# dusk-network/plonk

Hardware: NVIDIA H100
Metric: proofs/sec @ 2^16 gates (higher is better)
Workload: dtype u32 limbs (Fr 256-bit / Fp 384-bit Montgomery)

## Files before the change

plonk_b200/csrc/bigint.cuh:

```cuda
#pragma once
#include <stdint.h>

#if defined(__CUDACC__)
#define PB_HD __host__ __device__ __forceinline__
#define PB_D __device__ __forceinline__
#else
#define PB_HD inline
#define PB_D inline
#endif

#ifndef PB_SPLIT
#define PB_SPLIT 0
#endif

namespace pb {

#if defined(__CUDA_ARCH__)
#define PB_ASM2(name, ins)                                                         \
  PB_D uint32_t name(uint32_t a, uint32_t b) {                                     \
    uint32_t r;                                                                    \
    asm volatile(ins " %0, %1, %2;" : "=r"(r) : "r"(a), "r"(b));                   \
    return r;                                                                      \
  }
#define PB_ASM3(name, ins)                                                         \
// ... 81 lines not shown
#ifndef PB_FR_HYBRID
#define PB_FR_HYBRID 0
#endif
}
#if !defined(__CUDA_ARCH__)
#include <math.h>
#include <string.h>
#endif
namespace pb {
PB_HD double fma_rz(double a, double b, double c) {
#if defined(__CUDA_ARCH__)
  return __fma_rz(a, b, c);
#else
  return fma(a, b, c);
#endif
}
PB_HD uint64_t dbl_bits(double x) {
#if defined(__CUDA_ARCH__)
  return (uint64_t)__double_as_longlong(x);
#else
  uint64_t r;
  memcpy(&r, &x, 8);
  return r;
#endif
}
PB_HD double bits_dbl(uint32_t hi, uint32_t lo) {
#if defined(__CUDA_ARCH__)
  return __hiloint2double((int)hi, (int)lo);
#else
  const uint64_t r = ((uint64_t)hi << 32) | lo;
  double x;
  memcpy(&x, &r, 8);
  return x;
#endif
}

template <class P>
struct Field {
  static constexpr int N = P::N;
  uint32_t v[N];

  static PB_HD Field zero() {
    Field r;
#pragma unroll
    for (int i = 0; i < N; i++) r.v[i] = 0;
    return r;
  }
  static PB_HD Field one() {
    Field r;
#pragma unroll
    for (int i = 0; i < N; i++) r.v[i] = P::R1(i);
    return r;
  }
  static PB_HD Field r2() {
    Field r;
#pragma unroll
    for (int i = 0; i < N; i++) r.v[i] = P::R2(i);
    return r;
  }
  PB_HD bool is_zero() const {
    uint32_t x = 0;
#pragma unroll
    for (int i = 0; i < N; i++) x |= v[i];
    return x == 0;
  }
  PB_HD bool operator==(const Field& o) const {
    uint32_t x = 0;
#pragma unroll
    for (int i = 0; i < N; i++) x |= v[i] ^ o.v[i];
    return x == 0;
  }
  PB_HD bool operator!=(const Field& o) const { return !(*this == o); }

  static PB_HD void final_sub(uint32_t* r, const uint32_t* t, uint32_t hi) {
    uint32_t s[N];
    s[0] = sub_cc(t[0], P::MOD(0));
#pragma unroll
    for (int i = 1; i < N; i++) s[i] = subc_cc(t[i], P::MOD(i));
    uint32_t borrow = subc(hi, 0u);
    bool ge = (borrow == 0u);
#pragma unroll
    for (int i = 0; i < N; i++) r[i] = ge ? s[i] : t[i];
  }

  friend PB_HD Field operator+(const Field& a, const Field& b) {
    uint32_t t[N];
    t[0] = add_cc(a.v[0], b.v[0]);
#pragma unroll
    for (int i = 1; i < N; i++) t[i] = addc_cc(a.v[i], b.v[i]);
    uint32_t hi = addc(0u, 0u);
    Field r;
    final_sub(r.v, t, hi);
    return r;
  }
  friend PB_HD Field operator-(const Field& a, const Field& b) {
    uint32_t t[N];
    t[0] = sub_cc(a.v[0], b.v[0]);
#pragma unroll
    for (int i = 1; i < N; i++) t[i] = subc_cc(a.v[i], b.v[i]);
    uint32_t borrow = subc(0u, 0u);
    Field r;
    uint32_t m = borrow;
    r.v[0] = add_cc(t[0], P::MOD(0) & m);
#pragma unroll
    for (int i = 1; i < N - 1; i++) r.v[i] = addc_cc(t[i], P::MOD(i) & m);
    r.v[N - 1] = addc(t[N - 1], P::MOD(N - 1) & m);
    return r;
  }
  PB_HD Field neg() const { return zero() - *this; }
  PB_HD Field dbl() const { return *this + *this; }

  template <bool SPLIT, bool CIN, bool COUT>
  static PB_HD void link(uint32_t& lo, uint32_t& hi, uint32_t a, uint32_t b, uint32_t clo, uint32_t chi) {
    if (SPLIT)
      mad_pair_split<CIN, COUT>(lo, hi, a, b, clo, chi);
    else
      mad_pair<CIN, COUT>(lo, hi, a, b, clo, chi);
  }
  static PB_HD void mul_row(uint32_t* X, uint32_t* Y, const uint32_t* a, uint32_t bi) {
    constexpr bool S0 = (PB_SPLIT & 1) != 0, S1 = (PB_SPLIT & 2) != 0;
    Y[0] = add_cc(Y[0], X[1]);
#pragma unroll
    for (int k = 0; k < N - 2; k += 2) link<S0, true, true>(X[k], X[k + 1], a[k + 1], bi, X[k + 2], X[k + 3]);
    link<S0, true, false>(X[N - 2], X[N - 1], a[N - 1], bi, 0u, 0u);
    link<S1, false, true>(Y[0], Y[1], a[0], bi, Y[0], Y[1]);
#pragma unroll
    for (int j = 2; j < N; j += 2) link<S1, true, true>(Y[j], Y[j + 1], a[j], bi, Y[j], Y[j + 1]);
    X[N - 1] = addc(X[N - 1], 0u);
  }
  static PB_HD void acc_row(uint32_t* X, uint32_t* Y, const uint32_t* c, uint32_t di) {
    constexpr bool S0 = (PB_SPLIT & 1) != 0, S1 = (PB_SPLIT & 2) != 0;
    link<S0, false, true>(X[0], X[1], c[1], di, X[0], X[1]);
#pragma unroll
    for (int k = 2; k < N - 2; k += 2) link<S0, true, true>(X[k], X[k + 1], c[k + 1], di, X[k], X[k + 1]);
    link<S0, true, false>(X[N - 2], X[N - 1], c[N - 1], di, X[N - 2], X[N - 1]);
    link<S1, false, true>(Y[0], Y[1], c[0], di, Y[0], Y[1]);
#pragma unroll
    for (int j = 2; j < N; j += 2) link<S1, true, true>(Y[j], Y[j + 1], c[j], di, Y[j], Y[j + 1]);
    X[N - 1] = addc(X[N - 1], 0u);
  }
  static PB_HD void red_row(uint32_t* X , uint32_t* Y ) {
    constexpr bool S2 = (PB_SPLIT & 4) != 0, S3 = (PB_SPLIT & 8) != 0;
    const uint32_t m = mul_lo(Y[0], P::inv());
    link<S2, false, true>(X[0], X[1], P::MOD(1), m, X[0], X[1]);
#pragma unroll
    for (int k = 2; k < N - 2; k += 2) link<S2, true, true>(X[k], X[k + 1], P::MOD(k + 1), m, X[k], X[k + 1]);
    link<S2, true, false>(X[N - 2], X[N - 1], P::MOD(N - 1), m, X[N - 2], X[N - 1]);
    link<S3, false, true>(Y[0], Y[1], P::MOD(0), m, Y[0], Y[1]);
#pragma unroll
    for (int j = 2; j < N; j += 2) link<S3, true, true>(Y[j], Y[j + 1], P::MOD(j), m, Y[j], Y[j + 1]);
    X[N - 1] = addc(X[N - 1], 0u);
  }
  template <bool FIRST>
  static PB_HD void mont_row(uint32_t* X , uint32_t* Y ,
                             const uint32_t* a, uint32_t bi) {
    if (!FIRST) mul_row(X, Y, a, bi);
    red_row(X, Y);
  }

  friend PB_HD Field operator*(const Field& a, const Field& b) {
#if defined(__CUDA_ARCH__)
    if constexpr (P::HYBRID) return mul_hybrid(a, b);
#endif
    return mul_imad(a, b);
  }
  static PB_HD Field mul_imad(const Field& a, const Field& b) {
    uint32_t A[N], B[N];
    {
      const uint32_t bi = b.v[0];
#pragma unroll
      for (int j = 0; j < N; j += 2) {
        mul_pair(A[j], A[j + 1], a.v[j], bi);
        mul_pair(B[j], B[j + 1], a.v[j + 1], bi);
      }
      mont_row<true>(B, A, a.v, bi);
    }
#pragma unroll
    for (int i = 1; i < N - 1; i += 2) {
      mont_row<false>(A, B, a.v, b.v[i]);
      mont_row<false>(B, A, a.v, b.v[i + 1]);
    }
    mont_row<false>(A, B, a.v, b.v[N - 1]);
    uint32_t t[N];
    t[0] = add_cc(A[0], B[1]);
#pragma unroll
    for (int k = 1; k < N - 1; k++) t[k] = addc_cc(A[k], B[k + 1]);
    t[N - 1] = addc(A[N - 1], 0u);
    Field r;
    final_sub(r.v, t, 0u);
    return r;
  }
  template <int I>
  static PB_HD uint32_t sq_limb(const uint32_t* a, const uint32_t* a2, int k) {
    return k == I ? a[k] : (k == I + 1 ? (a[k] << 1) : a2[k]);
  }
  template <int I>
  static PB_HD void sqr_row(uint32_t* X, uint32_t* Y, const uint32_t* a, const uint32_t* a2) {
    constexpr bool S0 = (PB_SPLIT & 1) != 0, S1 = (PB_SPLIT & 2) != 0;
    const uint32_t bi = a[I];
    Y[0] = add_cc(Y[0], X[1]);
    constexpr int K0 = I & ~1;
#pragma unroll
    for (int k = 0; k < K0; k += 2) {
      X[k] = addc_cc(X[k + 2], 0u);
      X[k + 1] = addc_cc(X[k + 3], 0u);
    }
#pragma unroll
    for (int k = K0; k < N - 2; k += 2) link<S0, true, true>(X[k], X[k + 1], sq_limb<I>(a, a2, k + 1), bi, X[k + 2], X[k + 3]);
    link<S0, true, false>(X[N - 2], X[N - 1], sq_limb<I>(a, a2, N - 1), bi, 0u, 0u);
    constexpr int J0 = (I + 1) & ~1;
    if (J0 < N) {
      link<S1, false, true>(Y[J0], Y[J0 + 1], sq_limb<I>(a, a2, J0), bi, Y[J0], Y[J0 + 1]);
#pragma unroll
      for (int j = J0 + 2; j < N; j += 2) link<S1, true, true>(Y[j], Y[j + 1], sq_limb<I>(a, a2, j), bi, Y[j], Y[j + 1]);
      X[N - 1] = addc(X[N - 1], 0u);
    }
  }
  template <int I>
  static PB_HD void sqr_rows(uint32_t* A, uint32_t* B, const uint32_t* a, const uint32_t* a2) {
    if constexpr (I < N) {
      sqr_row<I>(A, B, a, a2);
      red_row(A, B);
      if constexpr (I + 1 < N) {
        sqr_row<I + 1>(B, A, a, a2);
        red_row(B, A);
      }
      sqr_rows<I + 2>(A, B, a, a2);
    }
  }
  PB_HD Field sqr() const {
#if defined(__CUDA_ARCH__)
    if constexpr (P::HYBRID && (P::MOD(N - 1) >> 30) == 0) return sqr_hybrid();
#endif
    if constexpr ((P::MOD(N - 1) >> 30) != 0) {
      return (*this) * (*this);
    } else {
      return sqr_half();
    }
  }
  PB_HD Field sqr_half() const {
    static_assert((P::MOD(N - 1) >> 30) == 0, "needs two spare bits in the top limb of the modulus");
    uint32_t a2[N];
    a2[0] = v[0] << 1;
#pragma unroll
    for (int k = 1; k < N; k++) a2[k] = (v[k] << 1) | (v[k - 1] >> 31);
    uint32_t A[N], B[N];
    {
      const uint32_t bi = v[0];
#pragma unroll
      for (int j = 0; j < N; j += 2) {
        mul_pair(A[j], A[j + 1], sq_limb<0>(v, a2, j), bi);
        mul_pair(B[j], B[j + 1], sq_limb<0>(v, a2, j + 1), bi);
      }
      red_row(B, A);
    }
    sqr_rows<1>(A, B, v, a2);
    uint32_t t[N];
    t[0] = add_cc(A[0], B[1]);
#pragma unroll
    for (int k = 1; k < N - 1; k++) t[k] = addc_cc(A[k], B[k + 1]);
    t[N - 1] = addc(A[N - 1], 0u);
    Field r;
    final_sub(r.v, t, 0u);
    return r;
  }

  static PB_HD Field mul2(const Field& a, const Field& b, const Field& c, const Field& d) {
#if defined(__CUDA_ARCH__)
    if constexpr (P::HYBRID) return mul2_hybrid(a, b, c, d);
#endif
    return mul2_imad(a, b, c, d);
  }
  static PB_HD Field mul2_imad(const Field& a, const Field& b, const Field& c, const Field& d) {
    static_assert((P::MOD(N - 1) >> 30) == 0, "mul2 needs two spare bits in the top limb of the modulus");
    uint32_t A[N], B[N];
    {
      const uint32_t bi = b.v[0];
#pragma unroll
      for (int j = 0; j < N; j += 2) {
        mul_pair(A[j], A[j + 1], a.v[j], bi);
        mul_pair(B[j], B[j + 1], a.v[j + 1], bi);
      }
      acc_row(B, A, c.v, d.v[0]);
      red_row(B, A);
    }
#pragma unroll
    for (int i = 1; i < N - 1; i += 2) {
      mul_row(A, B, a.v, b.v[i]);
      acc_row(A, B, c.v, d.v[i]);
      red_row(A, B);
      mul_row(B, A, a.v, b.v[i + 1]);
      acc_row(B, A, c.v, d.v[i + 1]);
      red_row(B, A);
    }
    mul_row(A, B, a.v, b.v[N - 1]);
    acc_row(A, B, c.v, d.v[N - 1]);
    red_row(A, B);
    uint32_t t[N];
    t[0] = add_cc(A[0], B[1]);
#pragma unroll
    for (int k = 1; k < N - 1; k++) t[k] = addc_cc(A[k], B[k + 1]);
    t[N - 1] = addc(A[N - 1], 0u);
    Field r;
    final_sub(r.v, t, 0u);
    return r;
  }
  static constexpr int L48 = (32 * N + 47) / 48;
  static constexpr int CUT_COL = (32 * N) / 48;
  static constexpr int CUT_SH = (32 * N) % 48;
  static constexpr int LAST_BITS = 32 * N - 48 * (L48 - 1);
  static PB_HD constexpr int npairs48(int k) { return k < 0 ? 0 : (k < L48 ? k + 1 : (k <= 2 * L48 - 2 ? 2 * L48 - 1 - k : 0)); }
  static PB_HD constexpr uint64_t col_off48(int k) {
    return (uint64_t)npairs48(k) * 0x4330000000000000ull + (uint64_t)npairs48(k - 1) * 0x4630000000000000ull;
  }
  static PB_HD uint32_t word_or_zero(const uint32_t* T, int k) { return k < 2 * N ? T[k] : 0u; }
  static PB_HD Field redc48(const uint32_t* T) {
    uint64_t c[2 * L48];
    const uint32_t gate = T[2 * N - 1] >> 30;
#pragma unroll
    for (int q = 0; q < L48; q++) {
      const uint32_t w0 = word_or_zero(T, 3 * q) | (q == 0 ? gate : 0u), w1 = word_or_zero(T, 3 * q + 1),
                     w2 = word_or_zero(T, 3 * q + 2);
      c[2 * q] = (uint64_t)w0 | ((uint64_t)(w1 & 0xffffu) << 32);
      c[2 * q + 1] = (uint64_t)((w1 >> 16) | (w2 << 16)) | ((uint64_t)(w2 >> 16) << 32);
    }
    const double C1 = 0x1p100, C2 = 0x1p100 + 0x1p52;
#pragma unroll
    for (int i = 0; i < L48; i++) {
      const uint32_t qlo = (uint32_t)c[i], qhi = (uint32_t)(c[i] >> 32);
      const uint64_t r = (uint64_t)qlo * P::inv48_lo();
      uint32_t rlo = (uint32_t)r, rhi = ((uint32_t)(r >> 32) + qlo * P::inv48_hi() + qhi * P::inv48_lo()) & 0xffffu;
      if (i == L48 - 1 && LAST_BITS < 48) {
        static_assert(LAST_BITS == 48 || LAST_BITS <= 32, "last step narrower than a word or a whole limb");
        rhi = 0;
        if (LAST_BITS < 32) rlo &= (1u << (LAST_BITS & 31)) - 1u;
      }
      const double m = bits_dbl(0x43300000u | rhi, rlo) - 0x1p52;
      double hi_prev = 0;
#pragma unroll
      for (int j = 0; j < L48; j++) {
        const double pj = (double)P::MOD48(j);
        const double hi = fma_rz(m, pj, C1);
        const double lo = fma_rz(m, pj, C2 - hi);
        if (j == 0)
          c[i] += dbl_bits(lo);
        else
          c[i + j] += dbl_bits(lo) + dbl_bits(hi_prev);
        hi_prev = hi;
      }
      c[i + L48] += dbl_bits(hi_prev);
      if (i < CUT_COL) c[i + 1] += (c[i] - col_off48(i)) >> 48;
    }
#pragma unroll
    for (int k = CUT_COL; k < 2 * L48; k++) c[k] -= col_off48(k);
#pragma unroll
    for (int k = CUT_COL; k < 2 * L48 - 1; k++) {
      c[k + 1] += c[k] >> 48;
      c[k] &= 0xffffffffffffull;
    }
    uint32_t t[N];
#pragma unroll
    for (int w = 0; w < N; w++) {
      const int s = CUT_SH + 32 * w, k = CUT_COL + s / 48, o = s % 48;
      if (o == 0)
        t[w] = (uint32_t)c[k];
      else if (o == 16)
        t[w] = (uint32_t)(c[k] >> 16);
      else
        t[w] = (uint32_t)(c[k] >> 32) | ((uint32_t)c[k + 1] << 16);
    }
    Field res;
    final_sub(res.v, t, 0u);
    return res;
  }
  static PB_HD void wide_top(uint32_t* T, const uint32_t* A, const uint32_t* B) {
    T[N] = add_cc(A[0], B[1]);
#pragma unroll
    for (int k = 1; k < N - 1; k++) T[N + k] = addc_cc(A[k], B[k + 1]);
    T[2 * N - 1] = addc(A[N - 1], 0u);
  }
  template <bool TWO>
  static PB_HD void wide_mul(uint32_t* T, const uint32_t* a, const uint32_t* b, const uint32_t* c, const uint32_t* d) {
    uint32_t A[N], B[N];
#pragma unroll
    for (int j = 0; j < N; j += 2) {
      mul_pair(A[j], A[j + 1], a[j], b[0]);
      mul_pair(B[j], B[j + 1], a[j + 1], b[0]);
    }
    if (TWO) acc_row(B, A, c, d[0]);
    T[0] = A[0];
#pragma unroll
    for (int i = 1; i < N; i += 2) {
      mul_row(A, B, a, b[i]);
      if (TWO) acc_row(A, B, c, d[i]);
      T[i] = B[0];
      if (i + 1 < N) {
        mul_row(B, A, a, b[i + 1]);
        if (TWO) acc_row(B, A, c, d[i + 1]);
        T[i + 1] = A[0];
      }
    }
    wide_top(T, A, B);
  }
  template <int I>
  static PB_HD void wide_sqr_rows(uint32_t* T, uint32_t* A, uint32_t* B, const uint32_t* a, const uint32_t* a2) {
    if constexpr (I < N) {
      sqr_row<I>(A, B, a, a2);
      T[I] = B[0];
      if constexpr (I + 1 < N) {
        sqr_row<I + 1>(B, A, a, a2);
        T[I + 1] = A[0];
      }
      wide_sqr_rows<I + 2>(T, A, B, a, a2);
    }
  }
  static PB_HD void wide_sqr(uint32_t* T, const uint32_t* v) {
    uint32_t a2[N];
    a2[0] = v[0] << 1;
#pragma unroll
    for (int k = 1; k < N; k++) a2[k] = (v[k] << 1) | (v[k - 1] >> 31);
    uint32_t A[N], B[N];
#pragma unroll
    for (int j = 0; j < N; j += 2) {
      mul_pair(A[j], A[j + 1], sq_limb<0>(v, a2, j), v[0]);
      mul_pair(B[j], B[j + 1], sq_limb<0>(v, a2, j + 1), v[0]);
    }
    T[0] = A[0];
    wide_sqr_rows<1>(T, A, B, v, a2);
    wide_top(T, A, B);
  }
  static PB_HD Field mul_hybrid(const Field& a, const Field& b) {
    uint32_t T[2 * N];
    wide_mul<false>(T, a.v, b.v, a.v, b.v);
    return redc48(T);
  }
  PB_HD Field sqr_hybrid() const {
    static_assert((P::MOD(N - 1) >> 30) == 0, "needs two spare bits in the top limb of the modulus");
    uint32_t T[2 * N];
    wide_sqr(T, v);
    return redc48(T);
  }
  static PB_HD Field mul2_hybrid(const Field& a, const Field& b, const Field& c, const Field& d) {
    static_assert((P::MOD(N - 1) >> 30) == 0, "needs two spare bits in the top limb of the modulus");
    uint32_t T[2 * N];
    wide_mul<true>(T, a.v, b.v, c.v, d.v);
    return redc48(T);
  }

  static PB_HD Field mul_sub(const Field& a, const Field& b, const Field& c, const Field& d) { return mul2(a, b, c.neg(), d); }


  PB_HD Field from_mont() const {
    Field o = zero();
    o.v[0] = 1;
    return (*this) * o;
  }
  PB_HD Field to_mont() const { return (*this) * r2(); }

  PB_HD Field pow(const uint32_t* e, int words) const {
    Field acc = one();
    bool started = false;
    for (int w = words - 1; w >= 0; w--) {
      for (int bit = 31; bit >= 0; bit--) {
        if (started) acc = acc.sqr();
        if ((e[w] >> bit) & 1u) {
          acc = started ? acc * (*this) : *this;
          started = true;
        }
      }
    }
    return acc;
  }
  PB_HD Field pow_u64(uint64_t e) const {
    uint32_t w[2] = {(uint32_t)e, (uint32_t)(e >> 32)};
    return pow(w, 2);
  }
  PB_HD Field inv() const {
    uint32_t e[N];
    e[0] = sub_cc(P::MOD(0), 2u);
#pragma unroll
    for (int i = 1; i < N; i++) e[i] = subc_cc(P::MOD(i), 0u);
    return pow(e, N);
  }
};

#define PB_LIMB_TABLE(name, n, ...)                     \
  static PB_HD constexpr uint32_t name(int i) {         \
    constexpr uint32_t T[n] = {__VA_ARGS__};            \
    return T[i];                                        \
  }

#if defined(__CUDACC__)
static __constant__ uint32_t c_fr_inv = 0xffffffffu;
#endif

struct FrParams {
  static constexpr int N = 8;
  static constexpr bool HYBRID = PB_FR_HYBRID != 0;
  static PB_HD constexpr uint64_t MOD48(int j) {
    constexpr uint64_t T[6] = {0xffff00000001ull, 0xfffe5bfeffffull, 0xd80553bda402ull, 0x3339d80809a1ull,
                               0xa753299d7d48ull, 0x73edull};
    return T[j];
  }
  static PB_HD constexpr uint32_t inv48_lo() { return 0xffffffffu; }
  static PB_HD constexpr uint32_t inv48_hi() { return 0xfffeu; }
  static PB_HD uint32_t inv() {
#if defined(__CUDA_ARCH__)
    return c_fr_inv;
#else
    return 0xffffffffu;
#endif
  }
  PB_LIMB_TABLE(MOD, 8, 0x00000001u, 0xffffffffu, 0xfffe5bfeu, 0x53bda402u, 0x09a1d805u, 0x3339d808u,
                0x299d7d48u, 0x73eda753u)
  PB_LIMB_TABLE(R1, 8, 0xfffffffeu, 0x00000001u, 0x00034802u, 0x5884b7fau, 0xecbc4ff5u, 0x998c4fefu,
                0xacc5056fu, 0x1824b159u)
  PB_LIMB_TABLE(R2, 8, 0xf3f29c6du, 0xc999e990u, 0x87925c23u, 0x2b6cedcbu, 0x7254398fu, 0x05d31496u,
                0x9f59ff11u, 0x0748d9d9u)
};

struct FpParams {
  static constexpr int N = 12;
  static constexpr bool HYBRID = PB_FP_HYBRID != 0;
  static PB_HD constexpr uint64_t MOD48(int j) {
    constexpr uint64_t T[8] = {0xffffffffaaabull, 0xb153ffffb9feull, 0xf6241eabfffeull, 0x6730d2a0f6b0ull,
                               0x4b84f38512bfull, 0x434bacd76477ull, 0xe69a4b1ba7b6ull, 0x1a0111ea397full};
    return T[j];
  }
  static PB_HD constexpr uint32_t inv48_lo() { return 0xfffcfffdu; }
  static PB_HD constexpr uint32_t inv48_hi() { return 0xfffcu; }
  static PB_HD uint32_t inv() { return 0xfffcfffdu; }
  PB_LIMB_TABLE(MOD, 12, 0xffffaaabu, 0xb9feffffu, 0xb153ffffu, 0x1eabfffeu, 0xf6b0f624u, 0x6730d2a0u,
                0xf38512bfu, 0x64774b84u, 0x434bacd7u, 0x4b1ba7b6u, 0x397fe69au, 0x1a0111eau)
  PB_LIMB_TABLE(R1, 12, 0x0002fffdu, 0x76090000u, 0xc40c0002u, 0xebf4000bu, 0x53c758bau, 0x5f489857u,
                0x70525745u, 0x77ce5853u, 0xa256ec6du, 0x5c071a97u, 0xfa80e493u, 0x15f65ec3u)
  PB_LIMB_TABLE(R2, 12, 0x1c341746u, 0xf4df1f34u, 0x09d104f1u, 0x0a76e6a6u, 0x4c95b6d5u, 0x8de5476cu,
                0x939d83c0u, 0x67eb88a9u, 0xb519952du, 0x9a793e85u, 0x92cae3aau, 0x11988fe5u)
};

typedef Field<FrParams> Fr;
typedef Field<FpParams> Fp;

}
```

plonk_b200/csrc/ecntt.cu:

```cuda
#include "common.cuh"
#include "ecntt.cuh"

namespace pb {

int get_twiddles(int logm, bool inverse, cudaStream_t st, const uint4** out);
Fr ntt_size_inv(int log_n);

namespace {

PB_D Fp ec_ld_fp(const uint4* q) {
  const uint4 a = q[0], b = q[1], c = q[2];
  Fp f;
  f.v[0] = a.x; f.v[1] = a.y; f.v[2] = a.z; f.v[3] = a.w;
  f.v[4] = b.x; f.v[5] = b.y; f.v[6] = b.z; f.v[7] = b.w;
  f.v[8] = c.x; f.v[9] = c.y; f.v[10] = c.z; f.v[11] = c.w;
  return f;
}
PB_D void ec_st_fp(uint4* q, const Fp& f) {
  q[0] = make_uint4(f.v[0], f.v[1], f.v[2], f.v[3]);
  q[1] = make_uint4(f.v[4], f.v[5], f.v[6], f.v[7]);
  q[2] = make_uint4(f.v[8], f.v[9], f.v[10], f.v[11]);
}
PB_D G1Xyzz ec_ld_xyzz(const uint4* p, size_t i) {
  G1Xyzz a;
  a.x = ec_ld_fp(p + 12 * i);
  a.y = ec_ld_fp(p + 12 * i + 3);
  a.zz = ec_ld_fp(p + 12 * i + 6);
  a.zzz = ec_ld_fp(p + 12 * i + 9);
  return a;
}
PB_D void ec_st_xyzz(uint4* p, size_t i, const G1Xyzz& a) {
  ec_st_fp(p + 12 * i, a.x);
  ec_st_fp(p + 12 * i + 3, a.y);
  ec_st_fp(p + 12 * i + 6, a.zz);
  ec_st_fp(p + 12 * i + 9, a.zzz);
}
PB_D Fr ec_ld_fr(const uint4* p, size_t i) {
  const uint4 a = p[2 * i], b = p[2 * i + 1];
  Fr f;
  f.v[0] = a.x; f.v[1] = a.y; f.v[2] = a.z; f.v[3] = a.w;
  f.v[4] = b.x; f.v[5] = b.y; f.v[6] = b.z; f.v[7] = b.w;
  return f;
}

__global__ void k_ec_load(const uint4* aff, size_t n, uint4* A) {
  const size_t i = (size_t)blockIdx.x * blockDim.x + threadIdx.x;
  if (i >= n) return;
  G1Affine p;
  p.x = ec_ld_fp(aff + 6 * i);
  p.y = ec_ld_fp(aff + 6 * i + 3);
  ec_st_xyzz(A, i, G1Xyzz::from_affine(p));
}

__global__ void __launch_bounds__(128) k_ec_stage(uint4* A, size_t n, int s, const uint4* tw) {
  const size_t t = (size_t)blockIdx.x * blockDim.x + threadIdx.x;
  if (t >= n / 2) return;
  const size_t len = n >> s, half = len >> 1;
  const size_t blk = t / half, j = t % half, i0 = blk * len + j, ex = j << s;
  G1Xyzz a = ec_ld_xyzz(A, i0), b = ec_ld_xyzz(A, i0 + half);
  ec_butterfly(a, b, ec_ld_fr(tw, ex), ex == 0);
  ec_st_xyzz(A, i0, a);
  ec_st_xyzz(A, i0 + half, b);
}

struct EcScalar {
  uint32_t k[8];
};
__global__ void __launch_bounds__(128) k_ec_finish(const uint4* A, size_t n, int log_n, EcScalar n_inv, uint4* out) {
  const size_t i = (size_t)blockIdx.x * blockDim.x + threadIdx.x;
  if (i >= n) return;
  const G1Affine r = xyzz_to_affine(xyzz_mul(ec_ld_xyzz(A, i), n_inv.k, 8));
  const size_t o = ec_bitrev((unsigned)i, log_n);
  ec_st_fp(out + 6 * o, r.x);
  ec_st_fp(out + 6 * o + 3, r.y);
}

}

int lagrange_key_dev(const uint4* d_in, int log_n, uint4* d_out, cudaStream_t st) {
  if (log_n < 0 || log_n > 28) return fail(PB200_ERR_INVALID_DOMAIN, "group-element NTT size");
  const size_t n = (size_t)1 << log_n;
  uint4* A = nullptr;
  PB_CUDA(cudaMalloc((void**)&A, n * 192));
  struct Free {
    uint4* p;
    ~Free() { cudaFree(p); }
  } guard{A};
  PB_LAUNCH(k_ec_load, div_up(n, 128), 128, 0, st, d_in, n, A);
  if (log_n > 0) {
    const uint4* tw = nullptr;
    PB_TRY(get_twiddles(log_n, true, st, &tw));
    for (int s = 0; s < log_n; s++) PB_LAUNCH(k_ec_stage, div_up(n / 2, 128), 128, 0, st, A, n, s, tw);
  }
  EcScalar ninv;
  const Fr c = ntt_size_inv(log_n).from_mont();
  for (int i = 0; i < 8; i++) ninv.k[i] = c.v[i];
  PB_LAUNCH(k_ec_finish, div_up(n, 128), 128, 0, st, (const uint4*)A, n, log_n, ninv, d_out);
  PB_CUDA(cudaGetLastError());
  PB_CUDA(stream_wait(st));
  return 0;
}

}
```

plonk_b200/csrc/g1.cuh:

```cuda
#pragma once
#include "bigint.cuh"

namespace pb {

struct G1Affine {
  Fp x, y;
  PB_HD bool is_inf() const { return x.is_zero() && y.is_zero(); }
};

struct G1Xyzz {
  Fp x, y, zz, zzz;
  static PB_HD G1Xyzz identity() {
    G1Xyzz r;
    r.x = Fp::zero();
    r.y = Fp::zero();
    r.zz = Fp::zero();
    r.zzz = Fp::zero();
    return r;
  }
  PB_HD bool is_inf() const { return zz.is_zero(); }
  static PB_HD G1Xyzz from_affine(const G1Affine& p) {
    G1Xyzz r;
    if (p.is_inf()) return identity();
    r.x = p.x;
    r.y = p.y;
    r.zz = Fp::one();
    r.zzz = Fp::one();
    return r;
  }
  PB_HD G1Xyzz neg() const {
    G1Xyzz r = *this;
    r.y = y.neg();
    return r;
  }
};

PB_HD G1Xyzz xyzz_dbl_affine(const Fp& x1, const Fp& y1) {
  G1Xyzz r;
  if (y1.is_zero()) return G1Xyzz::identity();
  Fp u = y1.dbl();
  Fp v = u.sqr();
  Fp w = u * v;
  Fp s = x1 * v;
  Fp xx = x1.sqr();
  Fp m = xx.dbl() + xx;
  r.x = m.sqr() - s.dbl();
  r.y = Fp::mul_sub(m, s - r.x, w, y1);
  r.zz = v;
  r.zzz = w;
  return r;
}

PB_HD G1Xyzz xyzz_dbl(const G1Xyzz& p) {
  if (p.is_inf()) return p;
  if (p.y.is_zero()) return G1Xyzz::identity();
  G1Xyzz r;
  Fp u = p.y.dbl();
  Fp v = u.sqr();
  Fp w = u * v;
  Fp s = p.x * v;
  Fp xx = p.x.sqr();
  Fp m = xx.dbl() + xx;
  r.x = m.sqr() - s.dbl();
  r.y = Fp::mul_sub(m, s - r.x, w, p.y);
  r.zz = v * p.zz;
  r.zzz = w * p.zzz;
  return r;
}

PB_HD void xyzz_madd(G1Xyzz& acc, const Fp& x2, const Fp& y2) {
  if (acc.is_inf()) {
    acc.x = x2;
    acc.y = y2;
    acc.zz = Fp::one();
    acc.zzz = Fp::one();
    return;
  }
  Fp u2 = x2 * acc.zz;
  Fp s2 = y2 * acc.zzz;
  Fp p = u2 - acc.x;
  Fp r = s2 - acc.y;
  if (p.is_zero()) {
    if (r.is_zero())
      acc = xyzz_dbl_affine(x2, y2);
    else
      acc = G1Xyzz::identity();
    return;
  }
  Fp pp = p.sqr();
  Fp ppp = p * pp;
  Fp q = acc.x * pp;
  Fp x3 = r.sqr() - ppp - q.dbl();
  Fp y3 = Fp::mul_sub(r, q - x3, acc.y, ppp);
  acc.x = x3;
  acc.y = y3;
  acc.zz = acc.zz * pp;
  acc.zzz = acc.zzz * ppp;
}

PB_HD void xyzz_add(G1Xyzz& acc, const G1Xyzz& o) {
  if (o.is_inf()) return;
  if (acc.is_inf()) {
    acc = o;
    return;
  }
  Fp u1 = acc.x * o.zz;
  Fp u2 = o.x * acc.zz;
  Fp s1 = acc.y * o.zzz;
  Fp s2 = o.y * acc.zzz;
  Fp p = u2 - u1;
  Fp r = s2 - s1;
  if (p.is_zero()) {
    if (r.is_zero())
      acc = xyzz_dbl(acc);
    else
      acc = G1Xyzz::identity();
    return;
  }
  Fp pp = p.sqr();
  Fp ppp = p * pp;
  Fp q = u1 * pp;
  Fp x3 = r.sqr() - ppp - q.dbl();
  Fp y3 = Fp::mul_sub(r, q - x3, s1, ppp);
  acc.x = x3;
  acc.y = y3;
  acc.zz = acc.zz * o.zz * pp;
  acc.zzz = acc.zzz * o.zzz * ppp;
}

PB_HD G1Xyzz xyzz_mul(const G1Xyzz& p, const uint32_t* k, int words) {
  G1Xyzz acc = G1Xyzz::identity();
  bool started = false;
  for (int w = words - 1; w >= 0; w--) {
    for (int bit = 31; bit >= 0; bit--) {
      if (started) acc = xyzz_dbl(acc);
      if ((k[w] >> bit) & 1u) {
        if (started) {
          xyzz_add(acc, p);
        } else {
          acc = p;
          started = true;
        }
      }
    }
  }
  return acc;
}

PB_HD G1Affine xyzz_to_affine(const G1Xyzz& p) {
  G1Affine r;
  if (p.is_inf()) {
    r.x = Fp::zero();
    r.y = Fp::zero();
    return r;
  }
  Fp i = (p.zz * p.zzz).inv();
  Fp izz = i * p.zzz;
  Fp izzz = i * p.zz;
  r.x = p.x * izz;
  r.y = p.y * izzz;
  return r;
}

}
```

plonk_b200/csrc/msm.cu:

```cuda
#include <algorithm>
#include <atomic>
#include <vector>

#include "common.cuh"
#include "fp_inv.cuh"
#include "g1.cuh"
#include "host_field.h"

struct pb200_srs {
  size_t n_points;
  int c;
  int W;
  uint4* table;
};

namespace pb {

static constexpr int kGroup = 8;
static constexpr unsigned kHeavyMin = 32, kHeavyFactor = 4;
static constexpr unsigned kHeavyChunk = 256, kHeavyChunkWide = 1024;

PB_D G1Affine ld_affine(const uint4* p, size_t i) {
  const uint4* q = p + 6 * i;
  uint4 a0 = __ldg(q), a1 = __ldg(q + 1), a2 = __ldg(q + 2), b0 = __ldg(q + 3), b1 = __ldg(q + 4), b2 = __ldg(q + 5);
  G1Affine r;
  r.x.v[0] = a0.x; r.x.v[1] = a0.y; r.x.v[2] = a0.z; r.x.v[3] = a0.w;
  r.x.v[4] = a1.x; r.x.v[5] = a1.y; r.x.v[6] = a1.z; r.x.v[7] = a1.w;
  r.x.v[8] = a2.x; r.x.v[9] = a2.y; r.x.v[10] = a2.z; r.x.v[11] = a2.w;
  r.y.v[0] = b0.x; r.y.v[1] = b0.y; r.y.v[2] = b0.z; r.y.v[3] = b0.w;
  r.y.v[4] = b1.x; r.y.v[5] = b1.y; r.y.v[6] = b1.z; r.y.v[7] = b1.w;
  r.y.v[8] = b2.x; r.y.v[9] = b2.y; r.y.v[10] = b2.z; r.y.v[11] = b2.w;
  return r;
}
PB_D void st_fp(uint4* q, const Fp& f) {
  q[0] = make_uint4(f.v[0], f.v[1], f.v[2], f.v[3]);
  q[1] = make_uint4(f.v[4], f.v[5], f.v[6], f.v[7]);
  q[2] = make_uint4(f.v[8], f.v[9], f.v[10], f.v[11]);
}
PB_D Fp ld_fp(const uint4* q) {
  uint4 a = q[0], b = q[1], c = q[2];
  Fp f;
  f.v[0] = a.x; f.v[1] = a.y; f.v[2] = a.z; f.v[3] = a.w;
  f.v[4] = b.x; f.v[5] = b.y; f.v[6] = b.z; f.v[7] = b.w;
  f.v[8] = c.x; f.v[9] = c.y; f.v[10] = c.z; f.v[11] = c.w;
  return f;
}
PB_D void st_affine(uint4* p, size_t i, const G1Affine& a) {
  st_fp(p + 6 * i, a.x);
  st_fp(p + 6 * i + 3, a.y);
}
PB_D void st_xyzz(uint4* p, size_t i, const G1Xyzz& a) {
  st_fp(p + 12 * i, a.x);
  st_fp(p + 12 * i + 3, a.y);
  st_fp(p + 12 * i + 6, a.zz);
  st_fp(p + 12 * i + 9, a.zzz);
}
PB_D G1Xyzz ld_xyzz(const uint4* p, size_t i) {
  G1Xyzz a;
  a.x = ld_fp(p + 12 * i);
  a.y = ld_fp(p + 12 * i + 3);
  a.zz = ld_fp(p + 12 * i + 6);
  a.zzz = ld_fp(p + 12 * i + 9);
  return a;
}

__global__ void k_msm_precompute(uint4* table, size_t n, int c, int W) {
  size_t i = (size_t)blockIdx.x * blockDim.x + threadIdx.x;
  if (i >= n) return;
  G1Affine p = ld_affine(table, i);
  for (int w = 1; w < W; w++) {
    if (!p.is_inf()) {
      G1Xyzz q = G1Xyzz::from_affine(p);
      for (int k = 0; k < c; k++) q = xyzz_dbl(q);
      p = xyzz_to_affine(q);
    }
    st_affine(table, (size_t)w * n + i, p);
  }
}

__global__ void __launch_bounds__(64) k_srs_setup(uint4* out, size_t n, Fr x, Fr g_scalar) {
  size_t i = (size_t)blockIdx.x * blockDim.x + threadIdx.x;
  if (i >= n) return;
  const Fr s = (g_scalar * x.pow_u64(i)).from_mont();
  G1Affine g;
  const uint32_t gx[12] = {0xfd530c16u, 0x5cb38790u, 0x9976fff5u, 0x7817fc67u, 0x143ba1c1u, 0x154f95c7u,
                           0xf3d0e747u, 0xf0ae6acdu, 0x21dbf440u, 0xedce6eccu, 0x9e0bfb75u, 0x12017741u};
  const uint32_t gy[12] = {0x0ce72271u, 0xbaac93d5u, 0x7918fd8eu, 0x8c22631au, 0x570725ceu, 0xdd595f13u,
                           0x50405194u, 0x51ac5829u, 0xad0059c0u, 0x0e1c8c3fu, 0x5008a26au, 0x0bbc3efcu};
#pragma unroll
  for (int k = 0; k < 12; k++) {
    g.x.v[k] = gx[k];
    g.y.v[k] = gy[k];
  }
  G1Xyzz acc = G1Xyzz::identity();
#pragma unroll 1
  for (int w = 7; w >= 0; w--) {
#pragma unroll 1
    for (int b = 31; b >= 0; b--) {
      acc = xyzz_dbl(acc);
      if ((s.v[w] >> b) & 1u) xyzz_madd(acc, g.x, g.y);
    }
  }
  st_affine(out, i, xyzz_to_affine(acc));
}

__global__ void __launch_bounds__(64) k_g1_decompress(const uint8_t* in, size_t n, int check_subgroup, uint4* out, unsigned* bad) {
  const size_t i = (size_t)blockIdx.x * blockDim.x + threadIdx.x;
  if (i >= n) return;
  const uint8_t* b = in + 48 * i;
  const unsigned flags = b[0];
  Fp x;
#pragma unroll
  for (int k = 0; k < 12; k++) {
    const int o = 44 - 4 * k;
    x.v[k] = ((uint32_t)b[o] << 24) | ((uint32_t)b[o + 1] << 16) | ((uint32_t)b[o + 2] << 8) | (uint32_t)b[o + 3];
  }
  x.v[11] &= 0x1fffffffu;
  bool ok = (flags & 0x80u) != 0;
  G1Affine pt;
  pt.x = Fp::zero();
  pt.y = Fp::zero();
  if (flags & 0x40u) {
    ok = ok && x.is_zero() && !(flags & 0x20u);
  } else {
    bool lt = false;
#pragma unroll
    for (int k = 11; k >= 0; k--) {
      const uint32_t m = FpParams::MOD(k);
      if (x.v[k] != m) {
        lt = x.v[k] < m;
        break;
      }
    }
    ok = ok && lt;
    if (ok) {
      const Fp xm = x.to_mont();
      const Fp four = Fp::one().dbl().dbl();
      const Fp y2 = xm.sqr() * xm + four;
      uint32_t e[12];
#pragma unroll
      for (int k = 0; k < 12; k++) e[k] = FpParams::MOD(k);
      e[0] += 1u;
#pragma unroll
      for (int k = 0; k < 12; k++) e[k] = (e[k] >> 2) | (k < 11 ? e[k + 1] << 30 : 0u);
      Fp y = y2.pow(e, 12);
// ... 1441 lines not shown
```

plonk_b200/csrc/verify.cu:

```cuda
#include <algorithm>
#include <mutex>
#include <thread>
#include <vector>

#include "common.cuh"
#include "g1.cuh"
#include "host_field.h"
#include "pairing.cuh"
#include "plonk_algebra.cuh"
#include "transcript.h"
#include "verify_scalars.h"

struct pb200_verifier {
  std::vector<uint8_t> label;
  uint64_t vk_n = 0;
  uint64_t size = 0, constraints = 0;
  uint8_t vk_comm[pb::N_POLY][48];
  uint8_t opening_key[PB200_OPENING_KEY_BYTES];
  std::vector<uint64_t> pi_idx;
  pb::VerifyKeyHost key;
  uint4* d_points = nullptr;
  pb::LineCoeffs* d_lines = nullptr;
};

namespace pb {
void g1_decompress_dev(const uint8_t* d_in, size_t n, uint4* d_out, unsigned* d_bad, cudaStream_t st);
int g1_decompress(const uint8_t* in, size_t n, int check_subgroup, uint8_t* out_raw);

namespace {
using pbh::HFr;

PB_D G1Affine ld_aff(const uint4* q) {
  G1Affine p;
  const uint32_t* w = (const uint32_t*)q;
#pragma unroll
  for (int k = 0; k < 12; k++) {
    p.x.v[k] = w[k];
    p.y.v[k] = w[12 + k];
  }
  return p;
}
PB_D void st_aff(uint4* q, const G1Affine& p) {
  uint32_t* w = (uint32_t*)q;
#pragma unroll
  for (int k = 0; k < 12; k++) {
    w[k] = p.x.v[k];
    w[12 + k] = p.y.v[k];
  }
}
PB_D G1Xyzz shfl_down_xyzz(const G1Xyzz& a, int d) {
  G1Xyzz r;
#pragma unroll
  for (int k = 0; k < 12; k++) {
    r.x.v[k] = __shfl_down_sync(0xffffffffu, a.x.v[k], d);
    r.y.v[k] = __shfl_down_sync(0xffffffffu, a.y.v[k], d);
    r.zz.v[k] = __shfl_down_sync(0xffffffffu, a.zz.v[k], d);
    r.zzz.v[k] = __shfl_down_sync(0xffffffffu, a.zzz.v[k], d);
  }
  return r;
}
PB_D G1Affine to_affine(const G1Xyzz& p) {
  if (p.is_inf()) return {Fp::zero(), Fp::zero()};
  const Fp i = fp_inv_bingcd(p.zz * p.zzz);
  return {p.x * (i * p.zzz), p.y * (i * p.zz)};
}

enum { P_A = 16, P_B, P_C, P_D, P_Z, P_TLOW, P_TMID, P_THIGH, P_TFOURTH, P_WZ, P_WZW };
__constant__ int c_term_point[32] = {0,  1,  2,  3,       4,      5,      7,       8,         9,    10, P_Z,   14, P_TLOW, P_TMID, P_THIGH, P_TFOURTH,
                                     P_A, P_B, P_C, P_D, 11, 12, 13, 6, 5, 1, 2, 15, P_WZ, P_WZW, -1, P_WZW};

__global__ void __launch_bounds__(128) k_verify_msm(const uint4* key_pts, const uint4* pts, const uint8_t* proof_comm,
                                                    const uint4* scalars, size_t n, int* status, uint4* out) {
  const size_t i = ((size_t)blockIdx.x * blockDim.x + threadIdx.x) >> 5;
  const int lane = threadIdx.x & 31;
  if (i >= n) return;
  bool bad = false;
  if (lane < 11) {
    const uint4* q = pts + 6 * (i * 11 + lane);
    const G1Affine p = ld_aff(q);
    if (p.is_inf()) {
      const uint8_t* e = proof_comm + 48 * (i * 11 + lane);
      uint32_t acc = e[0] ^ 0xc0u;
      for (int k = 1; k < 48; k++) acc |= e[k];
      bad = acc != 0;
    }
  }
  if (__any_sync(0xffffffffu, bad)) {
    if (lane == 0) status[i] = PB200_ERR_POINT_MALFORMED;
    return;
  }
  if (status[i] != PB200_OK) return;
  G1Xyzz acc = G1Xyzz::identity();
  const int src = c_term_point[lane];
  if (src >= 0) {
    const G1Affine p = src < 16 ? ld_aff(key_pts + 6 * src) : ld_aff(pts + 6 * (i * 11 + (src - 16)));
    if (!p.is_inf()) {
      const uint4* sp = scalars + 2 * (i * PB_VERIFY_TERMS + lane);
      const uint4 lo = sp[0], hi = sp[1];
      const uint32_t s[8] = {lo.x, lo.y, lo.z, lo.w, hi.x, hi.y, hi.z, hi.w};
#pragma unroll 1
      for (int w = 7; w >= 0; w--) {
#pragma unroll 1
        for (int b = 31; b >= 0; b--) {
          acc = xyzz_dbl(acc);
          if ((s[w] >> b) & 1u) xyzz_madd(acc, p.x, p.y);
        }
      }
    }
  }
  G1Xyzz left = G1Xyzz::identity();
  if (lane == 31) {
    const G1Affine wz = ld_aff(pts + 6 * (i * 11 + (P_WZ - 16)));
    left = acc;
    if (!wz.is_inf()) xyzz_madd(left, wz.x, wz.y);
    left = left.neg();
    acc = G1Xyzz::identity();
  }
#pragma unroll 1
  for (int d = 16; d >= 1; d >>= 1) {
    const G1Xyzz o = shfl_down_xyzz(acc, d);
    xyzz_add(acc, o);
  }
  if (lane == 0) st_aff(out + 12 * i + 6, to_affine(acc));
  if (lane == 31) st_aff(out + 12 * i, to_affine(left));
}

__global__ void __launch_bounds__(64) k_verify_pairing(const uint4* g1, const LineCoeffs* lines, size_t n, int* status) {
  const size_t i = (size_t)blockIdx.x * blockDim.x + threadIdx.x;
  if (i >= n || status[i] != PB200_OK) return;
  G1Affine p[2] = {ld_aff(g1 + 12 * i), ld_aff(g1 + 12 * i + 6)};
  const LineCoeffs* l[2] = {lines, lines + PB_G2_LINES};
  const Fp12 f = final_exponentiation(miller_loop2(p, l));
  status[i] = f.is_one() ? PB200_OK : PB200_ERR_VERIFY;
}

__global__ void k_g2_prepare(const uint8_t* enc, int count, LineCoeffs* lines, int* ok) {
  const int k = blockIdx.x * blockDim.x + threadIdx.x;
  if (k >= count) return;
  G2Affine q;
  const bool valid = g2_decode(enc + 96 * k, &q);
  ok[k] = !valid ? 0 : (q.inf ? 2 : 1);
  if (valid && !q.inf) g2_prepare(q, lines + (size_t)PB_G2_LINES * k);
}

__global__ void k_pairing_selftest(const uint4* g1, const LineCoeffs* lines, const int* ok, size_t n, uint32_t* out) {
  const size_t i = (size_t)blockIdx.x * blockDim.x + threadIdx.x;
  if (i >= n) return;
// ... 273 lines not shown
```

Measured before the change: 191.2.

## Use lazy-reduced Fp representation in XYZZ point arithmetic

Adds an FpR type holding Fp values in the range [0, 2p). Its Montgomery multiply, square and mul2 skip the final conditional subtraction, and add/sub reduce against 2p. G1Xyzz coordinates switch to FpR, so the EC add, madd and double formulas used by MSM, ECNTT and the verifier avoid one final subtraction per multiplication. Values are canonicalized on store and before affine conversion. Zero tests now must check both 0 and p, and correctness depends on the 8p < 2^384 headroom assumption.

Measured after the change: 197.8, median of 6. +3.4%, better.

```diff
diff --git a/plonk_b200/csrc/bigint.cuh b/plonk_b200/csrc/bigint.cuh
--- a/plonk_b200/csrc/bigint.cuh
+++ b/plonk_b200/csrc/bigint.cuh
@@ -187,6 +187,17 @@
 #pragma unroll
     for (int i = 0; i < N; i++) r[i] = ge ? s[i] : t[i];
   }
+  template <bool FULL>
+  static PB_HD Field finish(const uint32_t* t) {
+    Field r;
+    if (FULL) {
+      final_sub(r.v, t, 0u);
+    } else {
+#pragma unroll
+      for (int i = 0; i < N; i++) r.v[i] = t[i];
+    }
+    return r;
+  }
 
   friend PB_HD Field operator+(const Field& a, const Field& b) {
     uint32_t t[N];
@@ -263,12 +274,15 @@
     red_row(X, Y);
   }
 
-  friend PB_HD Field operator*(const Field& a, const Field& b) {
+  friend PB_HD Field operator*(const Field& a, const Field& b) { return mul<true>(a, b); }
+  template <bool FULL>
+  static PB_HD Field mul(const Field& a, const Field& b) {
 #if defined(__CUDA_ARCH__)
-    if constexpr (P::HYBRID) return mul_hybrid(a, b);
-#endif
-    return mul_imad(a, b);
-  }
+    if constexpr (P::HYBRID) return mul_hybrid<FULL>(a, b);
+#endif
+    return mul_imad<FULL>(a, b);
+  }
+  template <bool FULL = true>
   static PB_HD Field mul_imad(const Field& a, const Field& b) {
     uint32_t A[N], B[N];
     {
@@ -291,9 +305,7 @@
 #pragma unroll
     for (int k = 1; k < N - 1; k++) t[k] = addc_cc(A[k], B[k + 1]);
     t[N - 1] = addc(A[N - 1], 0u);
-    Field r;
-    final_sub(r.v, t, 0u);
-    return r;
+    return finish<FULL>(t);
   }
   template <int I>
   static PB_HD uint32_t sq_limb(const uint32_t* a, const uint32_t* a2, int k) {
@@ -333,16 +345,18 @@
       sqr_rows<I + 2>(A, B, a, a2);
     }
   }
+  template <bool FULL = true>
   PB_HD Field sqr() const {
 #if defined(__CUDA_ARCH__)
-    if constexpr (P::HYBRID && (P::MOD(N - 1) >> 30) == 0) return sqr_hybrid();
+    if constexpr (P::HYBRID && (P::MOD(N - 1) >> 30) == 0) return sqr_hybrid<FULL>();
 #endif
     if constexpr ((P::MOD(N - 1) >> 30) != 0) {
-      return (*this) * (*this);
+      return mul<FULL>(*this, *this);
     } else {
-      return sqr_half();
-    }
-  }
+      return sqr_half<FULL>();
+    }
+  }
+  template <bool FULL = true>
   PB_HD Field sqr_half() const {
     static_assert((P::MOD(N - 1) >> 30) == 0, "needs two spare bits in the top limb of the modulus");
     uint32_t a2[N];
@@ -365,17 +379,17 @@
 #pragma unroll
     for (int k = 1; k < N - 1; k++) t[k] = addc_cc(A[k], B[k + 1]);
     t[N - 1] = addc(A[N - 1], 0u);
-    Field r;
-    final_sub(r.v, t, 0u);
-    return r;
-  }
-
+    return finish<FULL>(t);
+  }
+
+  template <bool FULL = true>
   static PB_HD Field mul2(const Field& a, const Field& b, const Field& c, const Field& d) {
 #if defined(__CUDA_ARCH__)
-    if constexpr (P::HYBRID) return mul2_hybrid(a, b, c, d);
-#endif
-    return mul2_imad(a, b, c, d);
-  }
+    if constexpr (P::HYBRID) return mul2_hybrid<FULL>(a, b, c, d);
+#endif
+    return mul2_imad<FULL>(a, b, c, d);
+  }
+  template <bool FULL = true>
   static PB_HD Field mul2_imad(const Field& a, const Field& b, const Field& c, const Field& d) {
     static_assert((P::MOD(N - 1) >> 30) == 0, "mul2 needs two spare bits in the top limb of the modulus");
     uint32_t A[N], B[N];
@@ -406,9 +420,7 @@
 #pragma unroll
     for (int k = 1; k < N - 1; k++) t[k] = addc_cc(A[k], B[k + 1]);
     t[N - 1] = addc(A[N - 1], 0u);
-    Field r;
-    final_sub(r.v, t, 0u);
-    return r;
+    return finish<FULL>(t);
   }
   static constexpr int L48 = (32 * N + 47) / 48;
   static constexpr int CUT_COL = (32 * N) / 48;
@@ -419,6 +431,7 @@
     return (uint64_t)npairs48(k) * 0x4330000000000000ull + (uint64_t)npairs48(k - 1) * 0x4630000000000000ull;
   }
   static PB_HD uint32_t word_or_zero(const uint32_t* T, int k) { return k < 2 * N ? T[k] : 0u; }
+  template <bool FULL>
   static PB_HD Field redc48(const uint32_t* T) {
     uint64_t c[2 * L48];
     const uint32_t gate = T[2 * N - 1] >> 30;
@@ -474,9 +487,7 @@
       else
         t[w] = (uint32_t)(c[k] >> 32) | ((uint32_t)c[k + 1] << 16);
     }
-    Field res;
-    final_sub(res.v, t, 0u);
-    return res;
+    return finish<FULL>(t);
   }
   static PB_HD void wide_top(uint32_t* T, const uint32_t* A, const uint32_t* B) {
     T[N] = add_cc(A[0], B[1]);
@@ -534,22 +545,25 @@
     wide_sqr_rows<1>(T, A, B, v, a2);
     wide_top(T, A, B);
   }
+  template <bool FULL = true>
   static PB_HD Field mul_hybrid(const Field& a, const Field& b) {
     uint32_t T[2 * N];
     wide_mul<false>(T, a.v, b.v, a.v, b.v);
-    return redc48(T);
-  }
+    return redc48<FULL>(T);
+  }
+  template <bool FULL = true>
   PB_HD Field sqr_hybrid() const {
     static_assert((P::MOD(N - 1) >> 30) == 0, "needs two spare bits in the top limb of the modulus");
     uint32_t T[2 * N];
     wide_sqr(T, v);
-    return redc48(T);
-  }
+    return redc48<FULL>(T);
+  }
+  template <bool FULL = true>
   static PB_HD Field mul2_hybrid(const Field& a, const Field& b, const Field& c, const Field& d) {
     static_assert((P::MOD(N - 1) >> 30) == 0, "needs two spare bits in the top limb of the modulus");
     uint32_t T[2 * N];
     wide_mul<true>(T, a.v, b.v, c.v, d.v);
-    return redc48(T);
+    return redc48<FULL>(T);
   }
 
   static PB_HD Field mul_sub(const Field& a, const Field& b, const Field& c, const Field& d) { return mul2(a, b, c.neg(), d); }
@@ -646,4 +660,92 @@
 typedef Field<FrParams> Fr;
 typedef Field<FpParams> Fp;
 
-}
+struct FpR {
+  static constexpr int N = 12;
+  static_assert((FpParams::MOD(N - 1) >> 29) == 0, "FpR needs 8p < 2^384");
+  uint32_t v[N];
+
+  static PB_HD constexpr uint32_t MOD2(int i) {
+    return (FpParams::MOD(i) << 1) | (i > 0 ? FpParams::MOD(i - 1) >> 31 : 0u);
+  }
+  static PB_HD FpR from(const Fp& a) {
+    FpR r;
+#pragma unroll
+    for (int i = 0; i < N; i++) r.v[i] = a.v[i];
+    return r;
+  }
+  static PB_HD FpR zero() { return from(Fp::zero()); }
+  static PB_HD FpR one() { return from(Fp::one()); }
+  PB_HD Fp canonical() const {
+    Fp r;
+    Fp::final_sub(r.v, v, 0u);
+    return r;
+  }
+  PB_HD Fp raw() const {
+    Fp r;
+#pragma unroll
+    for (int i = 0; i < N; i++) r.v[i] = v[i];
+    return r;
+  }
+  PB_HD bool is_zero_limbs() const {
+    uint32_t x = 0;
+#pragma unroll
+    for (int i = 0; i < N; i++) x |= v[i];
+    return x == 0;
+  }
+  PB_HD bool is_zero_mod_p() const {
+    uint32_t z = 0, q = 0;
+#pragma unroll
+    for (int i = 0; i < N; i++) {
+      z |= v[i];
+      q |= v[i] ^ FpParams::MOD(i);
+    }
+    return z == 0 || q == 0;
+  }
+
+  friend PB_HD FpR operator+(const FpR& a, const FpR& b) {
+    uint32_t t[N], s[N];
+    t[0] = add_cc(a.v[0], b.v[0]);
+#pragma unroll
+    for (int i = 1; i < N; i++) t[i] = addc_cc(a.v[i], b.v[i]);
+    s[0] = sub_cc(t[0], MOD2(0));
+#pragma unroll
+    for (int i = 1; i < N; i++) s[i] = subc_cc(t[i], MOD2(i));
+    const bool ge = subc(0u, 0u) == 0u;
+    FpR r;
+#pragma unroll
+    for (int i = 0; i < N; i++) r.v[i] = ge ? s[i] : t[i];
+    return r;
+  }
+  friend PB_HD FpR operator-(const FpR& a, const FpR& b) {
+    uint32_t t[N];
+    t[0] = sub_cc(a.v[0], b.v[0]);
+#pragma unroll
+    for (int i = 1; i < N; i++) t[i] = subc_cc(a.v[i], b.v[i]);
+    const uint32_t m = subc(0u, 0u);
+    FpR r;
+    r.v[0] = add_cc(t[0], MOD2(0) & m);
+#pragma unroll
+    for (int i = 1; i < N - 1; i++) r.v[i] = addc_cc(t[i], MOD2(i) & m);
+    r.v[N - 1] = addc(t[N - 1], MOD2(N - 1) & m);
+    return r;
+  }
+  PB_HD FpR neg() const { return zero() - *this; }
+  PB_HD FpR dbl() const { return *this + *this; }
+
+  friend PB_HD FpR operator*(const FpR& a, const FpR& b) { return from(Fp::mul<false>(a.raw(), b.raw())); }
+  PB_HD FpR sqr() const { return from(raw().sqr<false>()); }
+  static PB_HD FpR mul2(const FpR& a, const FpR& b, const FpR& c, const FpR& d) {
+    return from(Fp::mul2<false>(a.raw(), b.raw(), c.raw(), d.raw()));
+  }
+  static PB_HD FpR mul_sub(const FpR& a, const FpR& b, const FpR& c, const FpR& d) {
+    Fp nc;
+    nc.v[0] = sub_cc(MOD2(0), c.v[0]);
+#pragma unroll
+    for (int i = 1; i < N - 1; i++) nc.v[i] = subc_cc(MOD2(i), c.v[i]);
+    nc.v[N - 1] = subc(MOD2(N - 1), c.v[N - 1]);
+    return from(Fp::mul2<false>(a.raw(), b.raw(), nc, d.raw()));
+  }
+};
+
+}
diff --git a/plonk_b200/csrc/ecntt.cu b/plonk_b200/csrc/ecntt.cu
--- a/plonk_b200/csrc/ecntt.cu
+++ b/plonk_b200/csrc/ecntt.cu
@@ -23,17 +23,18 @@
 }
 PB_D G1Xyzz ec_ld_xyzz(const uint4* p, size_t i) {
   G1Xyzz a;
-  a.x = ec_ld_fp(p + 12 * i);
-  a.y = ec_ld_fp(p + 12 * i + 3);
-  a.zz = ec_ld_fp(p + 12 * i + 6);
-  a.zzz = ec_ld_fp(p + 12 * i + 9);
+  a.x = FpR::from(ec_ld_fp(p + 12 * i));
+  a.y = FpR::from(ec_ld_fp(p + 12 * i + 3));
+  a.zz = FpR::from(ec_ld_fp(p + 12 * i + 6));
+  a.zzz = FpR::from(ec_ld_fp(p + 12 * i + 9));
   return a;
 }
 PB_D void ec_st_xyzz(uint4* p, size_t i, const G1Xyzz& a) {
-  ec_st_fp(p + 12 * i, a.x);
-  ec_st_fp(p + 12 * i + 3, a.y);
-  ec_st_fp(p + 12 * i + 6, a.zz);
-  ec_st_fp(p + 12 * i + 9, a.zzz);
+  const G1Xyzz c = a.canonical();
+  ec_st_fp(p + 12 * i, c.x.raw());
+  ec_st_fp(p + 12 * i + 3, c.y.raw());
+  ec_st_fp(p + 12 * i + 6, c.zz.raw());
+  ec_st_fp(p + 12 * i + 9, c.zzz.raw());
 }
 PB_D Fr ec_ld_fr(const uint4* p, size_t i) {
   const uint4 a = p[2 * i], b = p[2 * i + 1];
diff --git a/plonk_b200/csrc/g1.cuh b/plonk_b200/csrc/g1.cuh
--- a/plonk_b200/csrc/g1.cuh
+++ b/plonk_b200/csrc/g1.cuh
@@ -9,23 +9,23 @@
 };
 
 struct G1Xyzz {
-  Fp x, y, zz, zzz;
+  FpR x, y, zz, zzz;
   static PB_HD G1Xyzz identity() {
     G1Xyzz r;
-    r.x = Fp::zero();
-    r.y = Fp::zero();
-    r.zz = Fp::zero();
-    r.zzz = Fp::zero();
+    r.x = FpR::zero();
+    r.y = FpR::zero();
+    r.zz = FpR::zero();
+    r.zzz = FpR::zero();
     return r;
   }
-  PB_HD bool is_inf() const { return zz.is_zero(); }
+  PB_HD bool is_inf() const { return zz.is_zero_limbs(); }
   static PB_HD G1Xyzz from_affine(const G1Affine& p) {
     G1Xyzz r;
     if (p.is_inf()) return identity();
-    r.x = p.x;
-    r.y = p.y;
-    r.zz = Fp::one();
-    r.zzz = Fp::one();
+    r.x = FpR::from(p.x);
+    r.y = FpR::from(p.y);
+    r.zz = FpR::one();
+    r.zzz = FpR::one();
     return r;
   }
   PB_HD G1Xyzz neg() const {
@@ -33,19 +33,27 @@
     r.y = y.neg();
     return r;
   }
+  PB_HD G1Xyzz canonical() const {
+    G1Xyzz r;
+    r.x = FpR::from(x.canonical());
+    r.y = FpR::from(y.canonical());
+    r.zz = FpR::from(zz.canonical());
+    r.zzz = FpR::from(zzz.canonical());
+    return r;
+  }
 };
 
-PB_HD G1Xyzz xyzz_dbl_affine(const Fp& x1, const Fp& y1) {
+PB_HD G1Xyzz xyzz_dbl_affine(const FpR& x1, const FpR& y1) {
   G1Xyzz r;
-  if (y1.is_zero()) return G1Xyzz::identity();
-  Fp u = y1.dbl();
-  Fp v = u.sqr();
-  Fp w = u * v;
-  Fp s = x1 * v;
-  Fp xx = x1.sqr();
-  Fp m = xx.dbl() + xx;
+  if (y1.is_zero_mod_p()) return G1Xyzz::identity();
+  FpR u = y1.dbl();
+  FpR v = u.sqr();
+  FpR w = u * v;
+  FpR s = x1 * v;
+  FpR xx = x1.sqr();
+  FpR m = xx.dbl() + xx;
   r.x = m.sqr() - s.dbl();
-  r.y = Fp::mul_sub(m, s - r.x, w, y1);
+  r.y = FpR::mul_sub(m, s - r.x, w, y1);
   r.zz = v;
   r.zzz = w;
   return r;
@@ -53,45 +61,46 @@
 
 PB_HD G1Xyzz xyzz_dbl(const G1Xyzz& p) {
   if (p.is_inf()) return p;
-  if (p.y.is_zero()) return G1Xyzz::identity();
+  if (p.y.is_zero_mod_p()) return G1Xyzz::identity();
   G1Xyzz r;
-  Fp u = p.y.dbl();
-  Fp v = u.sqr();
-  Fp w = u * v;
-  Fp s = p.x * v;
-  Fp xx = p.x.sqr();
-  Fp m = xx.dbl() + xx;
+  FpR u = p.y.dbl();
+  FpR v = u.sqr();
+  FpR w = u * v;
+  FpR s = p.x * v;
+  FpR xx = p.x.sqr();
+  FpR m = xx.dbl() + xx;
   r.x = m.sqr() - s.dbl();
-  r.y = Fp::mul_sub(m, s - r.x, w, p.y);
+  r.y = FpR::mul_sub(m, s - r.x, w, p.y);
   r.zz = v * p.zz;
   r.zzz = w * p.zzz;
   return r;
 }
 
-PB_HD void xyzz_madd(G1Xyzz& acc, const Fp& x2, const Fp& y2) {
+PB_HD void xyzz_madd(G1Xyzz& acc, const Fp& x2c, const Fp& y2c) {
+  const FpR x2 = FpR::from(x2c), y2 = FpR::from(y2c);
   if (acc.is_inf()) {
     acc.x = x2;
     acc.y = y2;
-    acc.zz = Fp::one();
-    acc.zzz = Fp::one();
+    acc.zz = FpR::one();
+    acc.zzz = FpR::one();
     return;
   }
-  Fp u2 = x2 * acc.zz;
-  Fp s2 = y2 * acc.zzz;
-  Fp p = u2 - acc.x;
-  Fp r = s2 - acc.y;
-  if (p.is_zero()) {
-    if (r.is_zero())
+  FpR u2 = x2 * acc.zz;
+  FpR s2 = y2 * acc.zzz;
+  FpR p = u2 - acc.x;
+  FpR r = s2 - acc.y;
+  if (p.is_zero_mod_p()) {
+    if (r.is_zero_mod_p())
       acc = xyzz_dbl_affine(x2, y2);
     else
       acc = G1Xyzz::identity();
     return;
   }
-  Fp pp = p.sqr();
-  Fp ppp = p * pp;
-  Fp q = acc.x * pp;
-  Fp x3 = r.sqr() - ppp - q.dbl();
-  Fp y3 = Fp::mul_sub(r, q - x3, acc.y, ppp);
+  FpR pp = p.sqr();
+  FpR ppp = p * pp;
+  FpR q = acc.x * pp;
+  FpR x3 = r.sqr() - ppp - q.dbl();
+  FpR y3 = FpR::mul_sub(r, q - x3, acc.y, ppp);
   acc.x = x3;
   acc.y = y3;
   acc.zz = acc.zz * pp;
@@ -104,24 +113,24 @@
     acc = o;
     return;
   }
-  Fp u1 = acc.x * o.zz;
-  Fp u2 = o.x * acc.zz;
-  Fp s1 = acc.y * o.zzz;
-  Fp s2 = o.y * acc.zzz;
-  Fp p = u2 - u1;
-  Fp r = s2 - s1;
-  if (p.is_zero()) {
-    if (r.is_zero())
+  FpR u1 = acc.x * o.zz;
+  FpR u2 = o.x * acc.zz;
+  FpR s1 = acc.y * o.zzz;
+  FpR s2 = o.y * acc.zzz;
+  FpR p = u2 - u1;
+  FpR r = s2 - s1;
+  if (p.is_zero_mod_p()) {
+    if (r.is_zero_mod_p())
       acc = xyzz_dbl(acc);
     else
       acc = G1Xyzz::identity();
     return;
   }
-  Fp pp = p.sqr();
-  Fp ppp = p * pp;
-  Fp q = u1 * pp;
-  Fp x3 = r.sqr() - ppp - q.dbl();
-  Fp y3 = Fp::mul_sub(r, q - x3, s1, ppp);
+  FpR pp = p.sqr();
+  FpR ppp = p * pp;
+  FpR q = u1 * pp;
+  FpR x3 = r.sqr() - ppp - q.dbl();
+  FpR y3 = FpR::mul_sub(r, q - x3, s1, ppp);
   acc.x = x3;
   acc.y = y3;
   acc.zz = acc.zz * o.zz * pp;
@@ -154,11 +163,12 @@
     r.y = Fp::zero();
     return r;
   }
-  Fp i = (p.zz * p.zzz).inv();
-  Fp izz = i * p.zzz;
-  Fp izzz = i * p.zz;
-  r.x = p.x * izz;
-  r.y = p.y * izzz;
+  const Fp zz = p.zz.canonical(), zzz = p.zzz.canonical();
+  Fp i = (zz * zzz).inv();
+  Fp izz = i * zzz;
+  Fp izzz = i * zz;
+  r.x = p.x.canonical() * izz;
+  r.y = p.y.canonical() * izzz;
   return r;
 }
 
diff --git a/plonk_b200/csrc/msm.cu b/plonk_b200/csrc/msm.cu
--- a/plonk_b200/csrc/msm.cu
+++ b/plonk_b200/csrc/msm.cu
@@ -50,17 +50,18 @@
   st_fp(p + 6 * i + 3, a.y);
 }
 PB_D void st_xyzz(uint4* p, size_t i, const G1Xyzz& a) {
-  st_fp(p + 12 * i, a.x);
-  st_fp(p + 12 * i + 3, a.y);
-  st_fp(p + 12 * i + 6, a.zz);
-  st_fp(p + 12 * i + 9, a.zzz);
+  const G1Xyzz c = a.canonical();
+  st_fp(p + 12 * i, c.x.raw());
+  st_fp(p + 12 * i + 3, c.y.raw());
+  st_fp(p + 12 * i + 6, c.zz.raw());
+  st_fp(p + 12 * i + 9, c.zzz.raw());
 }
 PB_D G1Xyzz ld_xyzz(const uint4* p, size_t i) {
   G1Xyzz a;
-  a.x = ld_fp(p + 12 * i);
-  a.y = ld_fp(p + 12 * i + 3);
-  a.zz = ld_fp(p + 12 * i + 6);
-  a.zzz = ld_fp(p + 12 * i + 9);
+  a.x = FpR::from(ld_fp(p + 12 * i));
+  a.y = FpR::from(ld_fp(p + 12 * i + 3));
+  a.zz = FpR::from(ld_fp(p + 12 * i + 6));
+  a.zzz = FpR::from(ld_fp(p + 12 * i + 9));
   return a;
 }
 
diff --git a/plonk_b200/csrc/verify.cu b/plonk_b200/csrc/verify.cu
--- a/plonk_b200/csrc/verify.cu
+++ b/plonk_b200/csrc/verify.cu
@@ -61,8 +61,9 @@
 }
 PB_D G1Affine to_affine(const G1Xyzz& p) {
   if (p.is_inf()) return {Fp::zero(), Fp::zero()};
-  const Fp i = fp_inv_bingcd(p.zz * p.zzz);
-  return {p.x * (i * p.zzz), p.y * (i * p.zz)};
+  const Fp zz = p.zz.canonical(), zzz = p.zzz.canonical();
+  const Fp i = fp_inv_bingcd(zz * zzz);
+  return {p.x.canonical() * (i * zzz), p.y.canonical() * (i * zz)};
 }
 
 enum { P_A = 16, P_B, P_C, P_D, P_Z, P_TLOW, P_TMID, P_THIGH, P_TFOURTH, P_WZ, P_WZW };
```
